# mario-linov/graphs4cfd

Hardware: AMD Instinct MI355X
Metric: rollout timesteps/s (100k-node 2D mesh) (higher is better)
Workload: dtype f32 (MLP products: two-way fp16 split of both operands, 22 significand bits each, 3 partial products on the f16 MFMA pipe, fp32 accumulate; error vs fp64 within that of an fp32 GEMM)

## Files before the change

graphs4cfd_amd/_lib.py:

```python
from __future__ import annotations

import ctypes as C
import os
from typing import Optional

import torch

_HERE = os.path.dirname(os.path.abspath(__file__))
LIB_PATH = os.environ.get("G4C_LIB_PATH") or os.path.join(_HERE, "lib", "libg4c.so")

OK, EINVAL, ELAUNCH, EUNSUPPORTED = 0, -1, -2, -3
ACT_NONE, ACT_SELU, ACT_TANH = 0, 1, 2
MAX_SRC, MAX_LAYERS = 4, 4
MAX_HEADS = 2
NARROW_MAX = 8
KERNEL_MLP_RS = 5
KERNEL_MLP_RS2 = 6
KERNEL_MLP_BX6, KERNEL_MLP_WS = 2, 4
KERNEL_MLP_BX6_CERT, KERNEL_MLP_WS_CERT = 7, 8
KERNEL_MLP_WS_PRE = 9
KERNEL_NAMES = {0: "none", 1: "mlp_split_kernel", 2: "mlp_bx6_kernel", 3: "mlp_bx6i_kernel", 4: "mlp_ws_kernel", 5: "mlp_rs1_kernel", 6: "mlp_rs2_kernel",
                7: "mlp_bx6_kernel", 8: "mlp_ws_kernel", 9: "mlp_ws_kernel"}

TILE_SHAPE_GENERIC, TILE_SHAPE_NODE, TILE_SHAPE_UP, TILE_SHAPE_DOWN = 0, 1, 2, 3

_ACT_CODES = {None: ACT_NONE, "none": ACT_NONE, "selu": ACT_SELU, "tanh": ACT_TANH}


def act_code(activation) -> Optional[int]:
    if activation is None or isinstance(activation, str):
        return _ACT_CODES[activation]
    if activation is torch.tanh or activation is torch.nn.functional.tanh:
        return ACT_TANH
    if activation is torch.nn.functional.selu or activation is torch.selu:
        return ACT_SELU
    return None


class g4c_src_t(C.Structure):
    _fields_ = [("ptr", C.c_void_p), ("idx", C.c_void_p), ("width", C.c_int32), ("ld", C.c_int32),
                ("col0", C.c_int32), ("pre_act", C.c_int32), ("additive", C.c_int32), ("seg_mean", C.c_int32),
                ("w", C.c_void_p), ("seg_off", C.c_void_p), ("seg_perm", C.c_void_p), ("dtype", C.c_int32)]


class g4c_mlp_t(C.Structure):
    _fields_ = [("n_layers", C.c_int32), ("k_pad", C.c_int32 * MAX_LAYERS), ("n_pad", C.c_int32 * MAX_LAYERS),
                ("w", C.c_void_p * MAX_LAYERS), ("b", C.c_void_p * MAX_LAYERS),
                ("ln_gamma", C.c_void_p), ("ln_beta", C.c_void_p), ("ln_eps", C.c_float), ("n_out", C.c_int32), ("w_format", C.c_int32),
                ("range_slot", C.c_int32), ("range_certified", C.c_int32)]


WFMT_FP32, WFMT_F16X2, WFMT_BF16X3, WFMT_BF16_RS, WFMT_BF16_RS2, WFMT_BF16_RS2N, WFMT_BF16 = 0, 1, 2, 3, 4, 5, 6
DTYPE_F32, DTYPE_BF16 = 0, 1


# ... 124 lines not shown


class g4c_weighted_integrals_t(C.Structure):
    _fields_ = [("x", C.c_void_p), ("x_ld", C.c_int32), ("x_step", C.c_int32), ("sub", C.c_void_p), ("sub_ld", C.c_int32),
                ("sub_step", C.c_int32), ("nz", C.c_int32), ("w", C.c_void_p), ("step", C.c_void_p), ("t_host", C.c_int32),
                ("max_steps", C.c_int32), ("stats", C.c_void_p), ("scratch", C.c_void_p)]


SNAPSHOT_MAX_ROWS = 1024
SNAPSHOT_MAX_COLUMNS = 2 ** 31 - 1
SNAPSHOT_GRAM_BLOCK, SNAPSHOT_GRAM_CHUNK, SNAPSHOT_COMBINE_BLOCK = 64, 2048, 8


class g4c_snapshot_sel_t(C.Structure):
    _fields_ = [("rows", C.c_int32), ("first", C.c_int32), ("stride", C.c_int32), ("count", C.c_int32)]


_SIGNATURES = {
    "g4c_version": (C.c_int, []),
    "g4c_device_info": (C.c_int, [C.c_void_p, C.POINTER(C.c_int32), C.POINTER(C.c_int32)]),
    "g4c_last_error": (C.c_char_p, []),
    "g4c_plan_csr": (C.c_int, [C.c_void_p, C.c_int64, C.c_int64, C.c_void_p, C.c_void_p]),
    "g4c_plan_pool_edge": (C.c_int64, [C.c_void_p, C.c_int64, C.c_void_p, C.c_int64, C.c_void_p, C.c_void_p,
                                       C.c_void_p, C.c_void_p]),
    "g4c_plan_pool_edge_ordered": (C.c_int64, [C.c_void_p, C.c_int64, C.c_void_p, C.c_int64, C.c_int32, C.c_void_p, C.c_void_p,
                                               C.c_void_p, C.c_void_p]),
    "g4c_segment_reduce": (C.c_int, [C.c_void_p, C.c_int32, C.c_void_p, C.c_void_p, C.c_int32, C.c_int32, C.c_int32,
                                     C.c_int32, C.c_int32, C.c_void_p, C.c_int32, C.c_void_p]),
    "g4c_weighted_segment_mean": (C.c_int, [C.c_void_p, C.c_int32, C.c_void_p, C.c_void_p, C.c_void_p, C.c_int32,
                                            C.c_int32, C.c_void_p, C.c_int32, C.c_void_p, C.c_void_p]),
    "g4c_mlp_pack_layer": (C.c_int, [C.c_void_p, C.c_int32, C.c_int32, C.c_void_p, C.c_void_p, C.c_int32, C.c_int32, C.c_void_p,
                                     C.c_int32, C.c_int32, C.c_void_p]),
    "g4c_mlp_run": (C.c_int, [C.POINTER(g4c_mlp_t), C.POINTER(g4c_src_t), C.c_int32, C.c_int64, C.POINTER(g4c_mlp_io_t), C.c_void_p]),
    "g4c_plan_tiles": (C.c_int64, [C.c_void_p, C.c_int32, C.c_int32, C.c_void_p, C.c_void_p, C.c_int64]),
    "g4c_plan_row_ranges": (C.c_int64, [C.c_void_p, C.c_int32, C.c_int32, C.c_void_p, C.c_void_p, C.POINTER(C.c_int32)]),
    "g4c_mlp_ws_grid": (C.c_int, [C.c_void_p, C.POINTER(C.c_int32)]),
    "g4c_mlp_bx6i_enable": (C.c_int, [C.c_int]),
    "g4c_mlp_ws_enable": (C.c_int, [C.c_int]),
    "g4c_mlp_small_launch_tiles": (C.c_int, [C.c_int]),
    "g4c_layer_norm": (C.c_int, [C.c_void_p, C.c_int32, C.c_int64, C.c_int32, C.c_void_p, C.c_void_p, C.c_float, C.c_int32, C.c_void_p, C.c_int32, C.c_void_p]),
    "g4c_debug_mean_div": (C.c_int, [C.c_void_p, C.c_void_p, C.c_void_p, C.c_int64, C.c_void_p]),
    "g4c_mlp_last_kernel": (C.c_int, []),
    "g4c_mlp_last_row_ranges": (C.c_int, []),
    "g4c_mlp_shapes_enable": (C.c_int, [C.c_int]),
    "g4c_mlp_last_shape": (C.c_int, []),
    "g4c_mlp_tile_form": (C.c_int, [C.c_int]),
    "g4c_mlp_last_tile_rows": (C.c_int, []),
    "g4c_project_to_edges": (C.c_int, [C.c_void_p, C.c_int32, C.c_void_p, C.c_void_p, C.c_int64, C.c_int32,
                                       C.c_void_p, C.c_int32, C.c_void_p]),
    "g4c_edge_scalar_to_node_vector": (C.c_int, [C.c_void_p, C.c_int32, C.c_void_p, C.c_int32, C.c_int64, C.c_int32,
                                                 C.c_void_p, C.c_int32, C.c_void_p]),
    "g4c_knn_grid": (C.c_int, [C.c_void_p, C.c_void_p, C.c_void_p, C.c_void_p, C.c_int64, C.c_int32, C.c_void_p,
                               C.c_void_p, C.c_float, C.c_int32, C.c_void_p, C.c_void_p]),
    "g4c_knn_grid_query": (C.c_int, [C.c_void_p, C.c_void_p, C.c_void_p, C.c_int64, C.c_int32, C.c_void_p, C.c_void_p,
                                     C.c_float, C.c_void_p, C.c_void_p, C.c_int64, C.c_int32, C.c_void_p, C.c_void_p]),
    "g4c_knn_grid_periodic": (C.c_int, [C.c_void_p, C.c_void_p, C.c_void_p, C.c_int64, C.c_int32, C.POINTER(g4c_periodic_grid_t), C.c_int32,
                                        C.c_void_p, C.c_void_p]),
    "g4c_knn_grid_query_periodic": (C.c_int, [C.c_void_p, C.c_void_p, C.c_void_p, C.c_int64, C.c_int32, C.POINTER(g4c_periodic_grid_t),
                                              C.c_void_p, C.c_int64, C.c_int32, C.c_void_p, C.c_void_p]),
    "g4c_rollout_advance": (C.c_int, [C.c_void_p, C.c_int32, C.c_void_p, C.c_int32, C.c_void_p, C.c_int32,
                                      C.c_void_p, C.c_int64, C.c_void_p]),
    "g4c_rollout_record_scratch_doubles": (C.c_int64, [C.c_int64, C.c_int32]),
    "g4c_rollout_advance_record": (C.c_int, [C.c_void_p, C.c_int32, C.c_void_p, C.c_int32, C.POINTER(g4c_rollout_rec_t),
                                             C.c_void_p, C.c_int64, C.c_void_p]),
    "g4c_rollout_moments": (C.c_int, [C.c_void_p, C.c_int32, C.POINTER(g4c_rollout_moments_t), C.c_void_p, C.c_int64, C.c_void_p]),
    "g4c_rollout_spectrum": (C.c_int, [C.c_void_p, C.c_int32, C.POINTER(g4c_rollout_spectrum_t), C.c_void_p, C.c_int64, C.c_void_p]),
# ... 116 lines not shown
```

graphs4cfd_amd/csrc/mlp_common.h:

```cpp
#pragma once
#include "g4c_common.h"
#include <type_traits>

#ifndef G4C_ABLATE
#define G4C_ABLATE 0
#endif

namespace g4cm {

constexpr int KC = 32;
constexpr int XS = KC + 2;
constexpr int HS = 128 + 4;
constexpr int NP = 128;
constexpr int CHUNK_FLOATS = KC * NP;

typedef float f32x16 __attribute__((ext_vector_type(16)));
typedef float f32x8 __attribute__((ext_vector_type(8)));
typedef float f32x4 __attribute__((ext_vector_type(4)));
typedef float f32x2 __attribute__((ext_vector_type(2)));

struct Src {
    const float *ptr;
    const int *idx;
    int width, wpad, ld, col0, vec, pre_act;
// ... 259 lines not shown
    int io_n_tiles;
    bool deep_ring, shapes;
    int tile_form;
};
struct Ran { int kernel = G4C_KERNEL_NONE, shape = G4C_TILE_SHAPE_GENERIC, ranges = 0, tile_rows = 0; };

inline bool message_form(const Launch &L) {
    const Params &p = L.p;
    const Src &s = p.src[0];
    if (L.save || p.n_src != 1 || p.n_nar != 0 || (p.n_add != 0 && p.n_add != 2) || p.n_heads || p.n_out != NP || p.resid) return false;
    if (p.out_idx && (L.agg || !p.out)) return false;
    if (s.width != NP || !s.vec || s.seg_off) return false;
    for (int a = 0; a < p.n_add; ++a)
        if (p.add[a].width != NP || (p.add[a].ld & 3) || ((uintptr_t)p.add[a].ptr & (p.add[a].bf16 ? 7 : 15))) return false;
    if (p.out && !p.out_bf16 && ((p.out_ld & 3) || ((uintptr_t)p.out & 15))) return false;
    if (p.gamma && (((uintptr_t)p.gamma & 15) || ((uintptr_t)p.beta & 15))) return false;
    return ((uintptr_t)p.b & 15) == 0 && p.M < (1LL << 31);
}

bool split_takes(const Launch &L);
int split_launch(const Launch &L, hipStream_t st, Ran &ran);
bool tile_takes(const Launch &L);
int tile_launch(const Launch &L, hipStream_t st, Ran &ran);
bool bx6i_takes(const Launch &L);
int bx6i_launch(const Launch &L, hipStream_t st, Ran &ran);
bool ws_takes(const Launch &L);
bool ws_any_takes(const Launch &L);
bool ws_pre_takes(const Launch &L);
int ws_launch(const Launch &L, hipStream_t st, Ran &ran);
bool rs_takes(const Launch &L);
int rs_launch(const Launch &L, hipStream_t st, Ran &ran);
bool rs2_takes(const Launch &L);
int rs2_launch(const Launch &L, hipStream_t st, Ran &ran);

typedef unsigned u32x2 __attribute__((ext_vector_type(2)));
__device__ __forceinline__ f32x4 widen_bf16x4(u32x2 w) {
    f32x4 x;
    x[0] = __builtin_bit_cast(float, w[0] << 16); x[1] = __builtin_bit_cast(float, w[0] & 0xffff0000u);
    x[2] = __builtin_bit_cast(float, w[1] << 16); x[3] = __builtin_bit_cast(float, w[1] & 0xffff0000u);
    return x;
}


}
```

graphs4cfd_amd/csrc/mlp_run.hip:

```cpp
#include "mlp_common.h"
#include <atomic>
#include <climits>
using namespace g4cm;

namespace {

std::atomic<int> g_ws_mode{1};
std::atomic<int> g_bx6i_mode{1};
std::atomic<int> g_deep_tiles{512};
#ifndef G4C_TILE_SHAPES_DEFAULT
#define G4C_TILE_SHAPES_DEFAULT 1
#endif
std::atomic<int> g_shapes{G4C_TILE_SHAPES_DEFAULT};
#ifndef G4C_TILE_FORM_DEFAULT
#define G4C_TILE_FORM_DEFAULT 1
#endif
std::atomic<int> g_tile_form{G4C_TILE_FORM_DEFAULT};

constexpr long long WS_MIN_ROWS = 20000;
constexpr long long BX6I_MIN_ROWS = 400000;
constexpr long long TILE_ROWS64_FILL = 3;

int knob(std::atomic<int> &k, int value, int max_value) {
    const int prev = k.load(std::memory_order_relaxed);
// ... 301 lines not shown
                    "g4c_mlp_run: weights packed for the row-split update kernel (G4C_WFMT_BF16_RS2), launch outside its envelope");
        return rs2_launch;
    }
    if (at_size(g_ws_mode, WS_MIN_ROWS, L) && ws_takes(L)) return ws_launch;
    if (at_size(g_bx6i_mode, BX6I_MIN_ROWS, L) && bx6i_takes(L)) return bx6i_launch;
    return tile_takes(L) ? tile_launch : split_launch;
}

}

extern "C" int g4c_mlp_run(const g4c_mlp_t *mlp, const g4c_src_t *srcs, int32_t n_src, int64_t n_rows, const g4c_mlp_io_t *io,
                           void *stream) {
    g_last = Ran{};
    Launch L{};
    int rc;
    if ((rc = stage_call(mlp, srcs, n_src, n_rows, io, L))) return rc;
    if (n_rows == 0) return G4C_OK;
    g4c::DeviceGuard on_device(mlp->w[0]);
    if ((rc = stage_sources(srcs, n_src, mlp->k_pad[0], L))) return rc;
    if ((rc = stage_stream(mlp, L))) return rc;
    if ((rc = stage_outputs(io, L))) return rc;
    if ((rc = stage_save(io, L))) return rc;
    stage_range(mlp, io, L);
    if ((rc = stage_heads(io, L))) return rc;
    if (L.row_count == 0) return G4C_OK;
    if ((rc = stage_node(io, L))) return rc;
    L.p.n_tiles = (L.agg && !L.row_split && io->tile_rows) ? L.io_n_tiles : (int)((L.row_count + 31) / 32);
    const LaunchFn launch = choose(L);
    if (!launch) return G4C_EUNSUPPORTED;
    if (L.p.n_tiles == 0) return G4C_OK;
    return launch(L, (hipStream_t)stream, g_last);
}

extern "C" int g4c_mlp_ws_enable(int on) { return knob(g_ws_mode, on, 2); }
extern "C" int g4c_mlp_bx6i_enable(int on) { return knob(g_bx6i_mode, on, 2); }
extern "C" int g4c_mlp_small_launch_tiles(int n_tiles) { return knob(g_deep_tiles, n_tiles, INT_MAX); }
extern "C" int g4c_mlp_shapes_enable(int on) { return knob(g_shapes, on, 1); }
extern "C" int g4c_mlp_tile_form(int form) { return knob(g_tile_form, form, 1); }
extern "C" int g4c_mlp_last_tile_rows(void) { return g_last.tile_rows; }
extern "C" int g4c_mlp_last_kernel(void) { return g_last.kernel; }
extern "C" int g4c_mlp_last_shape(void) { return g_last.shape; }
extern "C" int g4c_mlp_last_row_ranges(void) { return g_last.ranges; }
```

graphs4cfd_amd/nn/blocks.py:

```python
from __future__ import annotations

from collections import OrderedDict
from dataclasses import dataclass
from typing import Callable, List, Optional, Sequence, Tuple

import torch
from torch import nn

from .. import _lib, ops, plan
from ..graph import Graph
from ..ops import Source

import os
HOIST_MIN_ROWS = 24576

Tensor = torch.Tensor


def _narrow_flags(sources: Sequence[Source]) -> List[bool]:
    return [s.width <= _lib.NARROW_MAX and s.index is None and s.pre_act == _lib.ACT_NONE and not s.additive for s in sources]


def _split_wide(sources: Sequence[Source]) -> List[Source]:
    if ops.grad_mode() or not any(s.width > 128 and not s.additive and s.segments is None for s in sources):
# ... 454 lines not shown
    n, k = int(edgeUnitVectorInverse.size(0)), int(edgeUnitVectorInverse.size(2))
    if edge_attr.size(0) != n * k:
        raise ValueError(f"{edge_attr.size(0)} edges cannot be viewed as {n} nodes x {k} incoming edges")
    return ops.edge_scalar_to_node_vector(edge_attr, edgeUnitVectorInverse, n, k)


COMPACT_MESSAGES = True
HOIST_BF16 = True
PRODUCTS_BF16 = True
ROW_SPLIT_BF16 = __import__('os').environ.get('G4C_ROW_SPLIT_BF16', '1') != '0'
AGGREGATE_BF16 = __import__('os').environ.get('G4C_AGGREGATE_BF16', '1') != '0'
COMPACT_LATENTS = __import__('os').environ.get('G4C_COMPACT_LATENTS', '1') != '0'
UPDATE_ROW_SPLIT = __import__('os').environ.get('G4C_UPDATE_ROW_SPLIT', '1') != '0'
RS1_MIN_ROWS = 20000


FUSE_LAYER = os.environ.get("G4C_FUSE_LAYER", "1") != "0"
FUSE_LAYER_MIN_ROWS = 2048
FUSE_LAYER_MAX_ROWS = 120_000


def will_fuse_layer(msg_mlp: MLP, upd_mlp: MLP, edge_index: Tensor, n_nodes: int) -> bool:
    if not FUSE_LAYER or ops.grad_mode() or ops.mlp_precision() != "f16x3":
        return False
    if not (FUSE_LAYER_MIN_ROWS <= int(edge_index.size(1)) < FUSE_LAYER_MAX_ROWS):
        return False
    lm, lu = msg_mlp._linears(), upd_mlp._linears()
    if len(lm) != len(lu) or len(lm) not in (2, 3) or any(l.out_features != 128 for l in lm + lu):
        return False
    if msg_mlp.input_size != 384 or upd_mlp.input_size != 256:
        return False
    _, csr = plan.edge_csr(edge_index, n_nodes)
    return csr.perm is None and csr.tiles() is not None


def _can_fuse_layer(msg_mlp: MLP, upd_mlp: MLP, v: Tensor, e, edge_index: Tensor, csr, v_src, n_targets, v_out, compact_messages: bool) -> bool:
    if v_src is not None or n_targets is not None or v_out is not None or compact_messages:
        return False
    if not will_fuse_layer(msg_mlp, upd_mlp, edge_index, int(v.size(0))):
        return False
    e_t = e.tensor if isinstance(e, Source) else e
    if isinstance(e, Source) and (e.index is not None or e.col0 != 0 or e.negate or e.segments is not None or e.additive):
        return False
    return int(v.size(1)) == 128 and int(e_t.size(1)) == 128 and e_t.dtype == torch.float32


def static_first_layer(msg_mlp: MLP, upd_mlp: MLP, e_src: Source, e_static, edge_index: Tensor, n_nodes: int, csr, hoists: bool) -> bool:
    if not (ops.STATIC_FIRST_LAYER and e_static and ops.StaticCache.active is not None and not ops.grad_mode() and hoists):
        return False
    if ops.mlp_precision() != "f16x3" or ops.effective_precision([128]) != "f16x3":
        return False
    lm = msg_mlp._linears()
    if len(lm) != 3 or any(l.out_features != 128 for l in lm) or msg_mlp.input_size != 384:
        return False
    if (e_src.pre_act != _lib.ACT_NONE or e_src.index is not None or e_src.col0 != 0 or e_src.negate or e_src.segments is not None
            or e_src.additive or e_src.width != 128 or e_src.tensor.dtype != torch.float32):
        return False
    if will_fuse_layer(msg_mlp, upd_mlp, edge_index, n_nodes):
        return False
    return ops.can_fuse_aggregation(csr, msg_mlp.output_size)


def _static_first_message(msg_mlp: MLP, e_src: Source, e_static, gathered, n_rows: int, products, gathered_bounds, product_bounds,
                          agg, store_rows: bool) -> Optional[Tensor]:
    H = 128
    first = ops.static_launch(STATIC_FIRST_NAME, list(e_static), lambda: ops.mlp_forward(
# ... 157 lines not shown
    def reset_parameters(self):
        for m in (self.node_mlp, self.edge_mlp):
            if m is not None and hasattr(m, 'reset_parameters'):
                m.reset_parameters()

    def step(self, v: Tensor, e: Tensor, edge_index: Tensor, act_code: int, e_pre_act: int = _lib.ACT_NONE,
             products: Optional[Sequence[Tensor]] = None, next_msg: Optional[MLP] = None, keep_e: bool = True,
             bounds: Optional[ops.RangeBounds] = None, e_static: Optional[Sequence[Tensor]] = None):
        return _mp_step(self.edge_mlp, self.node_mlp, v, e, edge_index, self.aggr, act_code, e_pre_act,
                        products=products, next_msg=next_msg, keep_e=keep_e, bounds=bounds, e_static=e_static)

    def forward(self, v: Tensor, e: Tensor, edge_index: Tensor, *, activation=None) -> Tuple[Tensor, Tensor]:
        return _public_mp(self.edge_mlp, self.node_mlp, v, e, edge_index, self.aggr, activation)


MP = GNBlock


class DownMP(nn.Module):

    def __init__(self, down_mlp_args: Tuple, hr_graph_idx: int):
        super().__init__()
        self.down_mlp = MLP(*down_mlp_args)
        self.hr_graph_idx = hr_graph_idx
        self.lr_graph_idx = hr_graph_idx + 1
        self.reset_parameters()

    def reset_parameters(self):
        for item in [self.down_mlp]:
            if hasattr(item, 'reset_parameters'):
                item.reset_parameters()

    def pool(self, graph: Graph, field: Tensor, edge_index: Tensor, edge_attr: Tensor, activation=None,
             e_pre_act: int = _lib.ACT_NONE, target_major: bool = False, bounds: Optional[ops.RangeBounds] = None):
        rb = bounds if bounds is not None else ops.RangeBounds()
        h, l = self.hr_graph_idx, self.lr_graph_idx
        rel = getattr(graph, f'e_{h}{l}')
        csr = plan.cluster_plan(getattr(graph, f'cluster_{l}'), getattr(graph, f'mask_{l}'))
        m = self.down_mlp.run([Source(rel), Source(field, bound=rb.v)], int(field.size(0)))
        m_bound = ops.take_bounds().out
        code = _lib.act_code(activation)
        pooled = ops.segment_reduce(m, csr, True, _lib.ACT_NONE if code is None else code)
        pooled = _finish(pooled, activation, code)
        pp = plan.pool_edge_plan(getattr(graph, f'idx{h}_to_idx{l}'), edge_index, target_major)
        ea_l = ops.segment_reduce(edge_attr, pp.csr, True, src_act=e_pre_act)
        rb.v = ops.act_bound(m_bound, code) if (activation is None or code is not None) else None
        rb.e, rb.products = ops.act_bound(rb.e, e_pre_act), None
        return pooled, pp.edge_index, ea_l

    def forward(self, graph: Graph, activation: Optional[Callable] = None) -> Graph:
        field, ei, ea = self.pool(graph, graph.field, graph.edge_index, graph.edge_attr, activation)
        graph.pos = getattr(graph, f'pos_{self.lr_graph_idx}')
        graph.field, graph.edge_index, graph.edge_attr = field, ei, ea
        return graph


class UpMP(nn.Module):

    def __init__(self, up_mlp_args: Tuple, lr_graph_idx: int):
        super().__init__()
        self.up_mlp = MLP(*up_mlp_args)
        self.lr_graph_idx = lr_graph_idx
        self.hr_graph_idx = lr_graph_idx - 1
        self.reset_parameters()

    def reset_parameters(self):
        for item in [self.up_mlp]:
            if hasattr(item, 'reset_parameters'):
                item.reset_parameters()

    def sources(self, graph: Graph, field_lr: Tensor, field_hr_old: Tensor,
                bounds: Tuple[Optional[float], Optional[float]] = (None, None)) -> List[Source]:
        h, l = self.hr_graph_idx, self.lr_graph_idx
        parent = plan.index32(getattr(graph, f'idx{h}_to_idx{l}'))
        return [Source(getattr(graph, f'e_{h}{l}'), negate=True), Source(field_lr, parent, bound=bounds[0]),
                Source(field_hr_old, bound=bounds[1])]

    def unpool(self, graph: Graph, field_lr: Tensor, field_hr_old: Tensor, activation=None) -> Tensor:
        return self.up_mlp.run(self.sources(graph, field_lr, field_hr_old), int(field_hr_old.size(0)), activation=activation)

# ... 104 lines not shown
```

graphs4cfd_amd/nn/mus_gnn.py:

```python
from __future__ import annotations

from typing import Optional

import torch

from .. import _lib, ops
from ..graph import Graph
from ..ops import Source
from . import blocks as _blocks
from .blocks import MLP, MP, DownMP, UpMP
from .model import GNN

SELU, TANH, NONE = _lib.ACT_SELU, _lib.ACT_TANH, _lib.ACT_NONE


class _MuSGNN(GNN):
    _PROGRAM: tuple = ()
    _PRETRAINED: dict = {}

    def __init__(self, model: str = None, *args, **kwargs) -> None:
        if model is not None:
            super().__init__(arch=None, weights=None, checkpoint=self._pretrained(self._PRETRAINED, model), *args, **kwargs)
        else:
            super().__init__(*args, **kwargs)
# ... 12 lines not shown
        self.node_decoder = MLP(*arch["decoder"])
        self.to(self.device)

    def _launch_for(self, mlp: MLP, sources, n_rows: int, act_code: int, k: int, edge_index: torch.Tensor):
        nxt = self._PROGRAM[k] if k < len(self._PROGRAM) else ""
        n_edges = int(edge_index.size(1))
        if nxt.startswith("mp") and (n_edges >= _blocks.HOIST_MIN_ROWS
                                     or _blocks.will_fuse_layer(getattr(self, nxt).edge_mlp, getattr(self, nxt).node_mlp, edge_index, n_rows)):
            cons = getattr(self, nxt).edge_mlp
            w = mlp.output_size
            res = mlp.run_with_heads(sources, n_rows, act_code, cons, cons.input_size - 2 * w, [w, w])
            if res is not None:
                return res
        return mlp.run_coded(sources, n_rows, act_code), None

    def forward(self, graph: Graph, t: Optional[int] = None) -> torch.Tensor:
        field0 = graph.field
        n = int(field0.size(0))
        inputs = [Source(getattr(graph, k)) for k in ('field', 'loc', 'glob', 'omega') if hasattr(graph, k)]
        edge_index = graph.edge_index
        e = ops.static_launch("edge_encoder", [graph.edge_attr],
                              lambda: self.edge_encoder.run_coded([Source(graph.edge_attr)], int(graph.edge_attr.size(0)), SELU))
        rb = ops.RangeBounds(e=ops.take_bounds().out)
        v, products = self._launch_for(self.node_encoder, inputs, n, SELU, 0, edge_index)
        lb = ops.take_bounds()
        rb.v, rb.products = lb.out, (lb.heads if products is not None else None)
        e_pending = NONE
        stash = []
        prog = self._PROGRAM
        for k, name in enumerate(prog):
            block = getattr(self, name)
            if name.startswith("down_mp"):
                stash.append((v, edge_index, e, e_pending, rb.v, rb.e))
                v, edge_index, e = block.pool(graph, v, edge_index, e, torch.tanh, e_pre_act=e_pending, target_major=True, bounds=rb)
                e_pending, products = NONE, None
            elif name.startswith("up_mp"):
                v_old, edge_index, e, e_pending, v_old_bound, rb.e = stash.pop()
                v, products = self._launch_for(block.up_mlp, block.sources(graph, v, v_old, (rb.v, v_old_bound)), int(v_old.size(0)), TANH,
                                               k + 1, edge_index)
                lb = ops.take_bounds()
                rb.v, rb.products = lb.out, (lb.heads if products is not None else None)
            else:
                nxt = prog[k + 1] if k + 1 < len(prog) else ""
                e_static = [graph.edge_attr] if k == 0 else None
                if nxt.startswith("mp"):
                    v, e, products = block.step(v, e, edge_index, SELU, e_pre_act=e_pending, products=products,
                                                next_msg=getattr(self, nxt).edge_mlp, bounds=rb, e_static=e_static)
                else:
                    drop_e = nxt.startswith("up_mp") or nxt == ""
                    v, e = block.step(v, e, edge_index, SELU, e_pre_act=e_pending, products=products, keep_e=not drop_e, bounds=rb,
                                      e_static=e_static)
                    products = None
                e_pending = SELU
        nf = self.num_fields
        return self.node_decoder.run_coded([Source(v)], n, NONE, resid=field0, resid_col0=int(field0.size(1)) - nf)


def _model(name: str, program: str, pretrained: dict, doc: str):
    cls = type(name, (_MuSGNN,), {"_PROGRAM": tuple(program.split()), "_PRETRAINED": pretrained, "__doc__": doc})
    cls.__module__ = __name__
    return cls


_DOC = """The {n}-GNN for {what} inference from Lino et al. (2022) (https://doi.org/10.1063/5.0097679)
(reference: nn/mus_gnn.py:{lines}).  `arch` keys: edge_encoder, node_encoder, {keys}, decoder — each MP entry
`((in, widths, layer_norm), (in, widths, layer_norm))`, each down/up entry `(in, widths, layer_norm)`."""

NsOneScaleGNN = _model(
# ... 49 lines not shown
```

graphs4cfd_amd/ops.py:

```python
from __future__ import annotations

import contextlib
import ctypes as C
import math
import os
from typing import List, Optional, Sequence, Tuple

import torch

from . import _lib
from ._args import Args, record_scratch_doubles
from .plan import CsrPlan

Tensor = torch.Tensor


class KernelTimer:
    active = None

    def __init__(self):
        self.records = []

    def __enter__(self):
        KernelTimer.active = self
# ... 2151 lines not shown
        _set_agg(io, csr, agg_out, agg_mean, ranges=packed.split == "f16x2" and save is None)
        if agg_out.dtype == torch.bfloat16:
            io.agg_mode |= 1 << 16
        out_b = 0 if not store_rows else packed.n_out * (2 if out.dtype == torch.bfloat16 else 4)
        nbytes = (in_bytes + out_b) * n_rows + 4.0 * packed.n_out * csr.n_seg
    if save is not None:
        live = [t for t in save if t is not None]
        _lib.require_hip(*live)
        if any(t.dim() != 2 or t.size(0) < n_rows or t.size(1) < 128 or t.stride(1) != 1 or _ld(t) != _ld(live[0]) for t in live):
            raise ValueError("save tensors must be [n_rows, >= 128] fp32 (or bf16) with one common leading dimension")
        if len(save) > _lib.MAX_LAYERS:
            raise ValueError(f"{len(save)} save tensors for {packed.desc.n_layers} layers")
        io.n_save, io.save_ld = len(save), _ld(live[0]) if live else 128
        io.save[:len(save)] = [_lib.ptr(t) for t in save]
        io.save_dtype = _rows_dtype("save", live)
        if mul is not None:
            lm = [t for t in mul if t is not None]
            _lib.require_hip(*lm)
            if len(mul) != len(save) or any(t.size(0) < n_rows or t.size(1) < 128 or t.stride(1) != 1 or _ld(t) != _ld(lm[0]) for t in lm):
                raise ValueError("mul tensors must be [n_rows, >= 128] fp32 (or bf16) with one common leading dimension, one entry per layer")
            io.mul[:len(mul)] = [_lib.ptr(t) for t in mul]
            io.mul_ld = _ld(lm[0]) if lm else 128
            io.mul_dtype = _rows_dtype("mul", lm)
        nbytes = (4.0 * (sum(packed.seg_widths) + packed.n_out) + 128.0 * sum(t.element_size() for t in live)) * n_rows
    lb = _certify(packed, sources, act, resid is not None or out_idx32 is not None or rows is not None, save is not None)
    try:
        _run(packed, arr, len(sources), n_rows, io, dev, packed.flops_per_row * row_count, nbytes)
    finally:
        packed.desc.range_certified = 0
    _last_bounds = lb
    if reduce_after is not None:
        segment_reduce(out, reduce_after[0], reduce_after[2], out=reduce_after[1])
    return out
```

include/g4c.h:

```cpp
#ifndef G4C_H
#define G4C_H

#include <stdint.h>

#ifdef __cplusplus
extern "C" {
#endif

#define G4C_OK 0
#define G4C_EINVAL (-1)
#define G4C_ELAUNCH (-2)
#define G4C_EUNSUPPORTED (-3)

#define G4C_ACT_NONE 0
#define G4C_ACT_SELU 1
#define G4C_ACT_TANH 2

#define G4C_MAX_SRC 4
#define G4C_MAX_LAYERS 4
#define G4C_MAX_HEADS 2
#define G4C_NARROW_MAX 8

int g4c_version(void);
int g4c_device_info(const void *device_ptr, int32_t *device , int32_t *cu_count );
// ... 96 lines not shown
    const void *mul[G4C_MAX_LAYERS];
    int32_t mul_ld;
    const g4c_mlp_t *upd;
    const float *v;
    int32_t v_ld, v_act;
    float *v_out;
    int32_t v_out_ld;
    int32_t *range_flag;
    int32_t save_dtype;
    int32_t mul_dtype;
    const int32_t *wg_rows, *wg_seg;
    int32_t n_wg, wg_pairs, wg_max_seg;
} g4c_mlp_io_t;

int g4c_mlp_run(const g4c_mlp_t *mlp , const g4c_src_t *srcs , int32_t n_src, int64_t n_rows,
                const g4c_mlp_io_t *io , void *stream);

int g4c_mlp_bx6i_enable(int on);

int g4c_mlp_ws_enable(int on);

int g4c_mlp_small_launch_tiles(int n_tiles);

#define G4C_KERNEL_NONE 0
#define G4C_KERNEL_MLP_SPLIT 1
#define G4C_KERNEL_MLP_BX6 2
#define G4C_KERNEL_MLP_BX6I 3
#define G4C_KERNEL_MLP_WS 4
#define G4C_KERNEL_MLP_RS 5
#define G4C_KERNEL_MLP_RS2 6
#define G4C_KERNEL_MLP_BX6_CERT 7
#define G4C_KERNEL_MLP_WS_CERT 8
#define G4C_KERNEL_MLP_WS_PRE 9
int g4c_mlp_last_kernel(void);
int g4c_mlp_last_row_ranges(void);

#define G4C_TILE_SHAPE_GENERIC 0
#define G4C_TILE_SHAPE_NODE 1
#define G4C_TILE_SHAPE_UP 2
#define G4C_TILE_SHAPE_DOWN 3
int g4c_mlp_shapes_enable(int on);
int g4c_mlp_last_shape(void);
int g4c_mlp_tile_form(int form);
int g4c_mlp_last_tile_rows(void);

int64_t g4c_plan_tiles(const int32_t *off , int32_t n_seg, int32_t max_rows, int32_t *tile_rows ,
                       int32_t *tile_seg , int64_t capacity);
int64_t g4c_plan_row_ranges(const int32_t *off , int32_t n_seg, int32_t n_wg, int32_t *wg_rows ,
                            int32_t *wg_seg , int32_t *max_seg );
int g4c_mlp_ws_grid(const void *device_ptr, int32_t *n_wg);

int g4c_layer_norm(const float *x, int32_t x_ld, int64_t n_rows, int32_t width, const float *gamma, const float *beta, float eps,
                   int32_t act, float *out, int32_t out_ld, void *stream);

int g4c_debug_mean_div(const float *a, const int32_t *count, float *out, int64_t n4, void *stream);

int g4c_project_to_edges(const float *v, int32_t v_ld, const int32_t *node, const float *unit,
                         int64_t n_edges, int32_t n_feat, float *out, int32_t out_ld, void *stream);

int g4c_edge_scalar_to_node_vector(const float *e, int32_t e_ld, const float *unit_inv, int32_t k,
                                   int64_t n_nodes, int32_t n_feat, float *out, int32_t out_ld,
                                   void *stream);

int g4c_knn_grid(const float *pos_sorted, const int32_t *cell_sorted, const int32_t *order,
                 const int32_t *cell_start, int64_t n, int32_t dim, const int32_t *n_cells, const float *origin,
                 float cell_size, int32_t k, int64_t *out, void *stream);

int g4c_knn_grid_query(const float *pos_sorted, const int32_t *order, const int32_t *cell_start, int64_t n, int32_t dim,
                       const int32_t *n_cells, const float *origin, float cell_size, const float *q_pos,
                       const int32_t *q_cell, int64_t m, int32_t k, int64_t *out, void *stream);

typedef struct g4c_periodic_grid {
    int32_t n_cells[3];
    float origin[3];
    float period[3];
    double cell[3];
} g4c_periodic_grid_t;
// ... 310 lines not shown
```

Before: 274.4.

## Fuse pooling segment-mean with next message MLP's node-side products

Adds a pool_products kernel that computes the pooled segment mean plus activation and, in the same launch, multiplies the pooled rows by the next message block's two 128x128 weight slices with split-fp16 MFMA. The MuS-GNN down-pool path passes the following mp block so its precomputed products can be reused. This removes a separate segment_reduce launch, an activation pass, and a re-read of pooled rows by the next edge MLP. In exchange it adds a specialised kernel with limited row parallelism per workgroup (32 segments per block) and more code paths gated by shape and precision checks.

```diff
diff --git a/graphs4cfd_amd/_lib.py b/graphs4cfd_amd/_lib.py
--- a/graphs4cfd_amd/_lib.py
+++ b/graphs4cfd_amd/_lib.py
@@ -19,8 +19,10 @@
 KERNEL_MLP_BX6, KERNEL_MLP_WS = 2, 4
 KERNEL_MLP_BX6_CERT, KERNEL_MLP_WS_CERT = 7, 8
 KERNEL_MLP_WS_PRE = 9
+KERNEL_POOL, KERNEL_POOL_CERT = 10, 11
 KERNEL_NAMES = {0: "none", 1: "mlp_split_kernel", 2: "mlp_bx6_kernel", 3: "mlp_bx6i_kernel", 4: "mlp_ws_kernel", 5: "mlp_rs1_kernel", 6: "mlp_rs2_kernel",
-                7: "mlp_bx6_kernel", 8: "mlp_ws_kernel", 9: "mlp_ws_kernel"}
+                7: "mlp_bx6_kernel", 8: "mlp_ws_kernel", 9: "mlp_ws_kernel",
+                10: "pool_products_kernel", 11: "pool_products_kernel"}
 
 TILE_SHAPE_GENERIC, TILE_SHAPE_NODE, TILE_SHAPE_UP, TILE_SHAPE_DOWN = 0, 1, 2, 3
 
@@ -211,6 +213,8 @@
     "g4c_mlp_pack_layer": (C.c_int, [C.c_void_p, C.c_int32, C.c_int32, C.c_void_p, C.c_void_p, C.c_int32, C.c_int32, C.c_void_p,
                                      C.c_int32, C.c_int32, C.c_void_p]),
     "g4c_mlp_run": (C.c_int, [C.POINTER(g4c_mlp_t), C.POINTER(g4c_src_t), C.c_int32, C.c_int64, C.POINTER(g4c_mlp_io_t), C.c_void_p]),
+    "g4c_pool_products": (C.c_int, [C.c_void_p, C.c_int32, C.c_void_p, C.c_void_p, C.c_int32, C.c_int32, C.c_void_p, C.c_int32,
+                                    C.POINTER(C.POINTER(g4c_mlp_t)), C.c_int32, C.POINTER(C.c_void_p), C.c_int32, C.c_void_p, C.c_void_p]),
     "g4c_plan_tiles": (C.c_int64, [C.c_void_p, C.c_int32, C.c_int32, C.c_void_p, C.c_void_p, C.c_int64]),
     "g4c_plan_row_ranges": (C.c_int64, [C.c_void_p, C.c_int32, C.c_int32, C.c_void_p, C.c_void_p, C.POINTER(C.c_int32)]),
     "g4c_mlp_ws_grid": (C.c_int, [C.c_void_p, C.POINTER(C.c_int32)]),
diff --git a/graphs4cfd_amd/csrc/mlp_common.h b/graphs4cfd_amd/csrc/mlp_common.h
--- a/graphs4cfd_amd/csrc/mlp_common.h
+++ b/graphs4cfd_amd/csrc/mlp_common.h
@@ -315,6 +315,9 @@
 int rs_launch(const Launch &L, hipStream_t st, Ran &ran);
 bool rs2_takes(const Launch &L);
 int rs2_launch(const Launch &L, hipStream_t st, Ran &ran);
+int pool_products_launch(const float *src, int32_t src_ld, const int32_t *perm, const int32_t *off, int32_t n_seg, int32_t act, float *out,
+                         int32_t out_ld, const g4c_mlp_t *const *heads, int32_t n_heads, float *const *head_out, int32_t head_ld,
+                         int32_t *range_flag, hipStream_t st, Ran &ran);
 
 typedef unsigned u32x2 __attribute__((ext_vector_type(2)));
 __device__ __forceinline__ f32x4 widen_bf16x4(u32x2 w) {
diff --git a/graphs4cfd_amd/csrc/mlp_run.hip b/graphs4cfd_amd/csrc/mlp_run.hip
--- a/graphs4cfd_amd/csrc/mlp_run.hip
+++ b/graphs4cfd_amd/csrc/mlp_run.hip
@@ -357,6 +357,14 @@
     return launch(L, (hipStream_t)stream, g_last);
 }
 
+extern "C" int g4c_pool_products(const float *src, int32_t src_ld, const int32_t *perm, const int32_t *off, int32_t n_seg, int32_t act,
+                                 float *out, int32_t out_ld, const g4c_mlp_t *const *heads, int32_t n_heads, float *const *head_out,
+                                 int32_t head_ld, int32_t *range_flag, void *stream) {
+    g_last = Ran{};
+    return pool_products_launch(src, src_ld, perm, off, n_seg, act, out, out_ld, heads, n_heads, head_out, head_ld, range_flag,
+                                (hipStream_t)stream, g_last);
+}
+
 extern "C" int g4c_mlp_ws_enable(int on) { return knob(g_ws_mode, on, 2); }
 extern "C" int g4c_mlp_bx6i_enable(int on) { return knob(g_bx6i_mode, on, 2); }
 extern "C" int g4c_mlp_small_launch_tiles(int n_tiles) { return knob(g_deep_tiles, n_tiles, INT_MAX); }
diff --git a/graphs4cfd_amd/csrc/pool_products.hip b/graphs4cfd_amd/csrc/pool_products.hip
--- /dev/null
+++ b/graphs4cfd_amd/csrc/pool_products.hip
@@ -0,0 +1,176 @@
+#include "mlp_common.h"
+#include <type_traits>
+
+using namespace g4cm;
+
+namespace {
+
+constexpr int POOL_ROWS = 32;
+#ifndef G4C_POOL_INFLIGHT
+#define G4C_POOL_INFLIGHT 4
+#endif
+constexpr int POOL_INFLIGHT = G4C_POOL_INFLIGHT;
+constexpr int POOL_PLN = POOL_ROWS * HB;
+
+struct PoolParams {
+    const float *src;
+    int src_ld;
+    const int *perm, *off;
+    int n_seg, act;
+    float *out;
+    int out_ld;
+    const float *w[G4C_MAX_HEADS];
+    float *head_out[G4C_MAX_HEADS];
+    int head_ld;
+    int *range_flag;
+    int range_slot;
+};
+
+struct PoolW { bf16x8 h[8], l[8]; };
+
+__device__ __forceinline__ void pool_load_w(PoolW &g, const float *w, unsigned lo_b) {
+    const __amdgpu_buffer_rsrc_t rs = __builtin_amdgcn_make_buffer_rsrc(const_cast<float *>(w), 0, 2 * BLOCK6, 0x00020000);
+#pragma unroll
+    for (int s = 0; s < 8; ++s) {
+        g.h[s] = ldw(rs, lo_b, 2u * s * STEP6);
+        g.l[s] = ldw(rs, lo_b + 1024u, 2u * s * STEP6);
+    }
+}
+
+template <int NH, bool TRACK>
+__global__ __launch_bounds__(256) void pool_products_kernel(const PoolParams p) {
+    __shared__ __attribute__((aligned(16))) __bf16 sB[2 * POOL_PLN];
+    const int tid = threadIdx.x;
+    const int lane = tid & 63;
+    const int wave = __builtin_amdgcn_readfirstlane(tid >> 6);
+    const int i = lane & 31, h = lane >> 5;
+    f16_range_mode();
+    typename std::conditional<TRACK, RangeS, RangeNone>::type rng;
+    const int row0 = blockIdx.x * POOL_ROWS;
+
+    const unsigned lo_b = 2u * (unsigned)(wave * 8 * STEP6 + lane * 8);
+    PoolW w;
+
+    const int grow_l = (lane >> 3) + 8 * wave, c4 = (lane & 7) * 4;
+    const int row = row0 + grow_l;
+    const bool live = row < p.n_seg;
+    const int beg = live ? p.off[row] : 0, end = live ? p.off[row + 1] : 0;
+    const float cnt = (float)((end - beg) > 1 ? (end - beg) : 1);
+    f32x4 a[4];
+#pragma unroll
+    for (int q = 0; q < 4; ++q) a[q] = f32x4{0.f, 0.f, 0.f, 0.f};
+    const float *sp = p.src + c4;
+    for (int r = beg; r < end; r += POOL_INFLIGHT) {
+        f32x4 v[POOL_INFLIGHT][4];
+#pragma unroll
+        for (int u = 0; u < POOL_INFLIGHT; ++u) {
+            const int pp = (r + u < end) ? r + u : end - 1;
+            const long long rr = p.perm ? p.perm[pp] : pp;
+#pragma unroll
+            for (int q = 0; q < 4; ++q) v[u][q] = *reinterpret_cast<const f32x4 *>(sp + rr * p.src_ld + q * KC);
+        }
+#pragma unroll
+        for (int u = 0; u < POOL_INFLIGHT; ++u) {
+            const bool on = r + u < end;
+#pragma unroll
+            for (int q = 0; q < 4; ++q)
+#pragma unroll
+                for (int e = 0; e < 4; ++e) a[q][e] += on ? v[u][q][e] : 0.f;
+        }
+    }
+    pool_load_w(w, p.w[0], lo_b);
+    __bf16 *d = sB + grow_l * HB + c4;
+#pragma unroll
+    for (int q = 0; q < 4; ++q) {
+        f32x4 x;
+#pragma unroll
+        for (int e = 0; e < 4; ++e) x[e] = g4c::apply_act(a[q][e] / cnt, p.act);
+        if (live) *reinterpret_cast<f32x4 *>(p.out + (long long)row * p.out_ld + q * KC + c4) = x;
+        bf16x4 vh, vl, unused;
+        split3x4<2>(x, vh, vl, unused, rng);
+        *reinterpret_cast<bf16x4 *>(d + q * KC) = vh;
+        *reinterpret_cast<bf16x4 *>(d + POOL_PLN + q * KC) = vl;
+    }
+    __syncthreads();
+
+    const __bf16 *pa = sB + i * HB + 8 * h;
+    const int fbase = wave * 32 + 4 * h;
+    const bool live_i = row0 + i < p.n_seg;
+    auto head = [&](float *ho, const float *next_w) __attribute__((always_inline)) {
+        const f32x16 zero16 = {0.f, 0.f, 0.f, 0.f, 0.f, 0.f, 0.f, 0.f, 0.f, 0.f, 0.f, 0.f, 0.f, 0.f, 0.f, 0.f};
+        f32x16 acc = zero16, acc1 = zero16;
+#pragma unroll
+        for (int s = 0; s < 8; ++s) {
+            const bf16x8 ah = *reinterpret_cast<const bf16x8 *>(pa + 16 * s), al = *reinterpret_cast<const bf16x8 *>(pa + POOL_PLN + 16 * s);
+            acc1 = mfma_f16(w.h[s], al, acc1);
+            acc1 = mfma_f16(w.l[s], ah, acc1);
+            acc = mfma_f16(w.h[s], ah, acc);
+        }
+        __builtin_amdgcn_sched_barrier(0);
+        if (next_w) pool_load_w(w, next_w, lo_b);
+        __builtin_amdgcn_sched_barrier(0);
+        float *hr = ho + (long long)(row0 + i) * p.head_ld + fbase;
+#pragma unroll
+        for (int gq = 0; gq < 4; ++gq) {
+            f32x4 x;
+#pragma unroll
+            for (int e = 0; e < 4; ++e) x[e] = fmaf(acc1[4 * gq + e], F16_LO_UNSCALE, acc[4 * gq + e]);
+            range_track(rng, x);
+            if (live_i) *reinterpret_cast<f32x4 *>(hr + 8 * gq) = x;
+        }
+    };
+    head(p.head_out[0], NH > 1 ? p.w[1] : nullptr);
+    if (NH > 1) head(p.head_out[1], nullptr);
+    if (TRACK && p.range_flag && range_hit(rng)) {
+        if (lane == 0) p.range_flag[p.range_slot] = 1;
+    }
+}
+
+bool aligned16(const void *q) { return ((uintptr_t)q & 15) == 0; }
+
+}
+
+namespace g4cm {
+
+int pool_products_launch(const float *src, int32_t src_ld, const int32_t *perm, const int32_t *off, int32_t n_seg, int32_t act, float *out,
+                         int32_t out_ld, const g4c_mlp_t *const *heads, int32_t n_heads, float *const *head_out, int32_t head_ld,
+                         int32_t *range_flag, hipStream_t st, Ran &ran) {
+    G4C_REQUIRE(n_seg >= 0 && src_ld >= NP && out_ld >= NP && head_ld >= NP && (src_ld & 3) == 0 && (out_ld & 3) == 0 && (head_ld & 3) == 0, G4C_EINVAL,
+                "g4c_pool_products: bad sizes n_seg=%d src_ld=%d out_ld=%d head_ld=%d (128-wide rows, strides multiples of 4)", n_seg, src_ld,
+                out_ld, head_ld);
+    G4C_REQUIRE(n_heads >= 1 && n_heads <= G4C_MAX_HEADS && heads && head_out, G4C_EINVAL, "g4c_pool_products: %d heads (1 .. %d)", n_heads,
+                G4C_MAX_HEADS);
+    G4C_REQUIRE(act >= 0 && act <= 2, G4C_EINVAL, "g4c_pool_products: bad activation %d", act);
+    if (n_seg == 0) return G4C_OK;
+    G4C_REQUIRE(off && out && aligned16(out) && aligned16(src), G4C_EINVAL, "g4c_pool_products: null or unaligned pointer");
+    G4C_REQUIRE(src != nullptr || perm == nullptr, G4C_EINVAL, "g4c_pool_products: null src with a permutation");
+    PoolParams p{};
+    p.src = src; p.src_ld = src_ld; p.perm = perm; p.off = off; p.n_seg = n_seg; p.act = act; p.out = out; p.out_ld = out_ld; p.head_ld = head_ld;
+    bool certified = true;
+    for (int hd = 0; hd < n_heads; ++hd) {
+        const g4c_mlp_t *m = heads[hd];
+        G4C_REQUIRE(m && m->w_format == G4C_WFMT_F16X2 && m->n_layers == 1 && m->k_pad[0] == NP && m->n_pad[0] == NP && m->n_out == NP && m->w[0] &&
+                        !m->ln_gamma && aligned16(m->w[0]),
+                    G4C_EUNSUPPORTED, "g4c_pool_products: head %d is not one bias-free 128 x 128 layer packed as G4C_WFMT_F16X2", hd);
+        G4C_REQUIRE(head_out[hd] && aligned16(head_out[hd]), G4C_EINVAL, "g4c_pool_products: head output %d is null or not 16-byte aligned", hd);
+        G4C_REQUIRE(m->range_slot >= 0, G4C_EINVAL, "g4c_pool_products: negative range_slot %d", m->range_slot);
+        p.w[hd] = (const float *)m->w[0]; p.head_out[hd] = head_out[hd];
+        certified = certified && m->range_certified;
+    }
+    p.range_flag = certified ? nullptr : range_flag;
+    p.range_slot = heads[0]->range_slot;
+    g4c::DeviceGuard on_device(out);
+    const dim3 grid((unsigned)((n_seg + POOL_ROWS - 1) / POOL_ROWS)), blk(256);
+    if (certified) {
+        if (n_heads == 1) pool_products_kernel<1, false><<<grid, blk, 0, st>>>(p);
+        else pool_products_kernel<2, false><<<grid, blk, 0, st>>>(p);
+    } else {
+        if (n_heads == 1) pool_products_kernel<1, true><<<grid, blk, 0, st>>>(p);
+        else pool_products_kernel<2, true><<<grid, blk, 0, st>>>(p);
+    }
+    ran.kernel = certified ? G4C_KERNEL_POOL_CERT : G4C_KERNEL_POOL;
+    ran.shape = G4C_TILE_SHAPE_GENERIC; ran.ranges = 0; ran.tile_rows = 0;
+    return g4c::check_launch("g4c_pool_products");
+}
+
+}
diff --git a/graphs4cfd_amd/nn/blocks.py b/graphs4cfd_amd/nn/blocks.py
--- a/graphs4cfd_amd/nn/blocks.py
+++ b/graphs4cfd_amd/nn/blocks.py
@@ -510,6 +510,15 @@
         return False
     _, csr = plan.edge_csr(edge_index, n_nodes)
     return csr.perm is None and csr.tiles() is not None
+
+
+def pools_products(down_mlp: MLP, next_mp: "GNBlock", edge_index_l: Tensor, n_coarse: int) -> bool:
+    if not ops.POOL_PRODUCTS or ops.grad_mode() or ops.mlp_precision() != "f16x3" or ops.effective_precision([128]) != "f16x3":
+        return False
+    msg = next_mp.edge_mlp
+    if down_mlp.output_size != 128 or msg.input_size != 384 or not msg.fits_one_launch() or msg._linears()[0].out_features != 128:
+        return False
+    return int(edge_index_l.size(1)) >= HOIST_MIN_ROWS or will_fuse_layer(msg, next_mp.node_mlp, edge_index_l, n_coarse)
 
 
 def _can_fuse_layer(msg_mlp: MLP, upd_mlp: MLP, v: Tensor, e, edge_index: Tensor, csr, v_src, n_targets, v_out, compact_messages: bool) -> bool:
@@ -733,7 +742,8 @@
                 item.reset_parameters()
 
     def pool(self, graph: Graph, field: Tensor, edge_index: Tensor, edge_attr: Tensor, activation=None,
-             e_pre_act: int = _lib.ACT_NONE, target_major: bool = False, bounds: Optional[ops.RangeBounds] = None):
+             e_pre_act: int = _lib.ACT_NONE, target_major: bool = False, bounds: Optional[ops.RangeBounds] = None,
+             next_mp: Optional["GNBlock"] = None):
         rb = bounds if bounds is not None else ops.RangeBounds()
         h, l = self.hr_graph_idx, self.lr_graph_idx
         rel = getattr(graph, f'e_{h}{l}')
@@ -741,12 +751,21 @@
         m = self.down_mlp.run([Source(rel), Source(field, bound=rb.v)], int(field.size(0)))
         m_bound = ops.take_bounds().out
         code = _lib.act_code(activation)
-        pooled = ops.segment_reduce(m, csr, True, _lib.ACT_NONE if code is None else code)
-        pooled = _finish(pooled, activation, code)
         pp = plan.pool_edge_plan(getattr(graph, f'idx{h}_to_idx{l}'), edge_index, target_major)
+        products, product_bounds = None, None
+        if next_mp is not None and code is not None and pools_products(self.down_mlp, next_mp, pp.edge_index, csr.n_seg):
+            H, msg = 128, next_mp.edge_mlp
+            pooled, products = ops.pool_products(m, csr, [msg._packed_cols(H * (1 + j), H * (2 + j), [H], [False], True) for j in range(2)],
+                                                 code, src_bound=m_bound)
+            product_bounds = ops.take_bounds().heads
+        else:
+            pooled = ops.segment_reduce(m, csr, True, _lib.ACT_NONE if code is None else code)
+            pooled = _finish(pooled, activation, code)
         ea_l = ops.segment_reduce(edge_attr, pp.csr, True, src_act=e_pre_act)
         rb.v = ops.act_bound(m_bound, code) if (activation is None or code is not None) else None
-        rb.e, rb.products = ops.act_bound(rb.e, e_pre_act), None
+        rb.e, rb.products = ops.act_bound(rb.e, e_pre_act), product_bounds
+        if next_mp is not None:
+            return pooled, pp.edge_index, ea_l, products
         return pooled, pp.edge_index, ea_l
 
     def forward(self, graph: Graph, activation: Optional[Callable] = None) -> Graph:
diff --git a/graphs4cfd_amd/nn/mus_gnn.py b/graphs4cfd_amd/nn/mus_gnn.py
--- a/graphs4cfd_amd/nn/mus_gnn.py
+++ b/graphs4cfd_amd/nn/mus_gnn.py
@@ -68,8 +68,13 @@
             block = getattr(self, name)
             if name.startswith("down_mp"):
                 stash.append((v, edge_index, e, e_pending, rb.v, rb.e))
-                v, edge_index, e = block.pool(graph, v, edge_index, e, torch.tanh, e_pre_act=e_pending, target_major=True, bounds=rb)
-                e_pending, products = NONE, None
+                nxt = prog[k + 1] if k + 1 < len(prog) else ""
+                kw = dict(e_pre_act=e_pending, target_major=True, bounds=rb)
+                if nxt.startswith("mp"):
+                    v, edge_index, e, products = block.pool(graph, v, edge_index, e, torch.tanh, next_mp=getattr(self, nxt), **kw)
+                else:
+                    (v, edge_index, e), products = block.pool(graph, v, edge_index, e, torch.tanh, **kw), None
+                e_pending = NONE
             elif name.startswith("up_mp"):
                 v_old, edge_index, e, e_pending, v_old_bound, rb.e = stash.pop()
                 v, products = self._launch_for(block.up_mlp, block.sources(graph, v, v_old, (rb.v, v_old_bound)), int(v_old.size(0)), TANH,
diff --git a/graphs4cfd_amd/ops.py b/graphs4cfd_amd/ops.py
--- a/graphs4cfd_amd/ops.py
+++ b/graphs4cfd_amd/ops.py
@@ -2207,3 +2207,73 @@
     if reduce_after is not None:
         segment_reduce(out, reduce_after[0], reduce_after[2], out=reduce_after[1])
     return out
+
+
+POOL_PRODUCTS = os.environ.get("G4C_POOL_PRODUCTS", "1") != "0"
+
+
+def pool_products(src: Tensor, csr: CsrPlan, heads: Sequence[PackedMLP], act: int = _lib.ACT_NONE, out: Optional[Tensor] = None,
+                  head_outs: Optional[Sequence[Tensor]] = None, src_bound: Optional[float] = None) -> Tuple[Tensor, List[Tensor]]:
+    global _last_bounds
+    _last_bounds = None
+    a = Args("pool_products", TypeError)
+    a.strided_rows(src, "src", cols=128)
+    _csr_arg(csr, "csr")
+    act = _act_arg(act, "act")
+    if torch.is_grad_enabled() and src.requires_grad:
+        raise NotImplementedError("pool_products is an inference-only form; call under torch.no_grad() or use segment_reduce and mlp_forward")
+    if csr.perm is None and int(src.size(0)) < csr.n:
+        raise ValueError(f"src: the plan reads rows 0 .. {csr.n - 1}, got shape {tuple(src.shape)}")
+    if csr.perm is not None and csr.n > 0 and int(src.size(0)) == 0:
+        raise ValueError(f"src: the plan reads {csr.n} rows through its permutation, got shape {tuple(src.shape)}")
+    heads = list(heads)
+    if not 1 <= len(heads) <= _lib.MAX_HEADS:
+        raise ValueError(f"heads: pool_products: expected 1 .. {_lib.MAX_HEADS} packed layers, got {len(heads)}")
+    for j, pk in enumerate(heads):
+        if (pk.split != "f16x2" or pk.desc.n_layers != 1 or pk.seg_widths != (128,) or pk.n_out != 128 or pk.n_heads or any(pk.narrow)
+                or pk.desc.ln_gamma or pk.params[1][0] is not None):
+            raise NotImplementedError(f"heads[{j}]: pool_products: one bias-free 128 x 128 layer packed for f16x3, no LayerNorm")
+    named = [("src", src)]
+    if out is not None:
+        a.strided_rows(out, "out", cols=128)
+        named.append(("out", out))
+    if head_outs is not None:
+        if len(head_outs) != len(heads):
+            raise ValueError(f"head_outs: pool_products: {len(head_outs)} outputs for {len(heads)} heads")
+        for j, t in enumerate(head_outs):
+            a.strided_rows(t, f"head_outs[{j}]", cols=128)
+            named.append((f"head_outs[{j}]", t))
+    for name, t in named[1:]:
+        if int(t.size(0)) < csr.n_seg:
+            raise ValueError(f"{name}: pool_products: expected at least {csr.n_seg} rows, got shape {tuple(t.shape)}")
+    dev = _lib.require_hip(src, csr.off, csr.perm, out, *(head_outs or ()))
+    if any(pk.device != dev for pk in heads):
+        raise RuntimeError(f"MLP weights on {heads[0].device}, inputs on {dev}")
+    if out is None:
+        out = torch.empty((csr.n_seg, 128), dtype=torch.float32, device=dev)
+    if head_outs is None:
+        head_outs = [torch.empty((csr.n_seg, 128), dtype=torch.float32, device=dev) for _ in heads]
+    head_outs = list(head_outs)
+    for name, t in [("src", src), ("out", out)] + [(f"head_outs[{j}]", t) for j, t in enumerate(head_outs)]:
+        if _ld(t) % 4 or t.data_ptr() % 16:
+            raise ValueError(f"{name}: pool_products: needs 16-byte aligned rows (row stride a multiple of 4), got {_ld(t)} at {t.data_ptr():#x}")
+    if any(_ld(t) != _ld(head_outs[0]) for t in head_outs):
+        raise ValueError("head_outs: pool_products: the heads share one row stride")
+    out_bound = act_bound(src_bound, act)
+    certified = bool(RANGE_PROOFS and certifies(out_bound))
+    lb = LaunchBounds(out_bound, out_bound, None if out_bound is None else [pk.norms["w0"][0] * out_bound for pk in heads])
+    descs = (C.POINTER(_lib.g4c_mlp_t) * len(heads))(*[C.pointer(pk.desc) for pk in heads])
+    outs = (C.c_void_p * len(heads))(*[t.data_ptr() for t in head_outs])
+    n = csr.n_seg
+    nbytes = 4.0 * (128 * (csr.n + n * (1 + len(heads))) + n + 1 + (csr.n if csr.perm is not None else 0))
+    for pk in heads:
+        pk.desc.range_certified = 1 if certified else 0
+    try:
+        _timed("pool_products_kernel", sum(pk.flops_per_row for pk in heads) * n, nbytes, lambda: _lib.check(_lib.load().g4c_pool_products(
+            _lib.ptr(src), _ld(src), _lib.ptr(csr.perm), _lib.ptr(csr.off), n, act, _lib.ptr(out), _ld(out), descs, len(heads), outs,
+            _ld(head_outs[0]), _launch_flags(dev).data_ptr(), _lib.stream_handle(dev))))
+    finally:
+        for pk in heads:
+            pk.desc.range_certified = 0
+    _last_bounds = lb
+    return out, head_outs
diff --git a/include/g4c.h b/include/g4c.h
--- a/include/g4c.h
+++ b/include/g4c.h
@@ -152,6 +152,8 @@
 #define G4C_KERNEL_MLP_BX6_CERT 7
 #define G4C_KERNEL_MLP_WS_CERT 8
 #define G4C_KERNEL_MLP_WS_PRE 9
+#define G4C_KERNEL_POOL 10
+#define G4C_KERNEL_POOL_CERT 11
 int g4c_mlp_last_kernel(void);
 int g4c_mlp_last_row_ranges(void);
 
@@ -163,6 +165,10 @@
 int g4c_mlp_last_shape(void);
 int g4c_mlp_tile_form(int form);
 int g4c_mlp_last_tile_rows(void);
+
+int g4c_pool_products(const float *src, int32_t src_ld, const int32_t *perm, const int32_t *off, int32_t n_seg, int32_t act,
+                      float *out, int32_t out_ld, const g4c_mlp_t *const *heads, int32_t n_heads, float *const *head_out,
+                      int32_t head_ld, int32_t *range_flag, void *stream);
 
 int64_t g4c_plan_tiles(const int32_t *off , int32_t n_seg, int32_t max_rows, int32_t *tile_rows ,
                        int32_t *tile_seg , int64_t capacity);
```

After: 275.7 (median of 6 runs). Within noise of the previous version (+0.5%).
